# Rainbowboys/fm_spark

Measured on AMD Instinct MI355X. Metric: FM SGD train samples/sec at k=16, 1/8 GPUs; % of HBM roofline, higher is better.
Workload: dtype f32; 1 GPU; c3: synthetic hashed 100M features, 39 nnz/row, k=16, batch 256K; num_features=100000000, k=16, batch_rows_per_gpu=262144, global_batch=262144, launch=single

## Files before the change

### fm_spark_amd/csrc/fm_context.h

```cpp
#pragma once

#include <map>
#include <memory>
#include <utility>

#include "fm_internal.h"

namespace fmhip {

struct Pinned {
  void* p = nullptr;
  size_t bytes = 0;
  void ensure(size_t n) {
    if (n <= bytes && p) return;
    if (p) (void)hipHostFree(p);
    p = nullptr;
    FM_HIP_CHECK(hipHostMalloc(&p, n, hipHostMallocDefault));
    bytes = n;
  }
  void ensure_slack(size_t n) {
    if (n > bytes || !p) ensure(n + n / 8 + 4096);
  }
  ~Pinned() {
    if (p) (void)hipHostFree(p);
// ... 217 lines not shown
      }
      it->second.ms += ms;
      it->second.n += 1;
      free_events.push_back(pe.second.first);
      free_events.push_back(pe.second.second);
    }
    pending.clear();
  }

  void ensure_hist(int64_t need) {
    if (need <= hist_cap) return;
    int64_t c = std::max<int64_t>(4096, hist_cap);
    while (c < need) c *= 2;
    FM_HIP_CHECK(hipStreamSynchronize(stream));
    DevBuf nb;
    nb.ensure(sizeof(double) * 3 * c);
    FM_HIP_CHECK(hipMemset(nb.p, 0, sizeof(double) * 3 * c));
    if (hist_cap > 0)
      FM_HIP_CHECK(hipMemcpy(nb.p, loss_hist.p, sizeof(double) * 3 * hist_cap, hipMemcpyDeviceToDevice));
    loss_hist = std::move(nb);
    hist_cap = c;
  }

  ~fm_ctx() {
    group.reset();
    (void)hipSetDevice(cfg.device);
    if (stream) (void)hipStreamSynchronize(stream);
    if (copy_stream) (void)hipStreamSynchronize(copy_stream);
    for (auto& h : hslot) {
      if (h.copied) (void)hipEventDestroy(h.copied);
      if (h.consumed) (void)hipEventDestroy(h.consumed);
    }
    if (copy_stream) (void)hipStreamDestroy(copy_stream);
    for (auto& pe : pending) {
      (void)hipEventDestroy(pe.second.first);
      (void)hipEventDestroy(pe.second.second);
    }
    for (auto e : free_events) (void)hipEventDestroy(e);
    if (side) (void)hipStreamSynchronize(side);
    if (ev_fork) (void)hipEventDestroy(ev_fork);
    if (ev_join) (void)hipEventDestroy(ev_join);
    if (ev_upd_done) (void)hipEventDestroy(ev_upd_done);
    if (side_own) (void)hipStreamSynchronize(side_own);
    if (side_own) (void)hipStreamDestroy(side_own);
    rec.release();
    loss_hist.release();
    DevBuf* bufs[] = {&work.S, &work.yl, &work.loss_part, &work.part, &work.ucnt,
                      &work.sort.keys_a, &work.sort.keys_b, &work.sort.vals_a, &work.sort.vals_b,
                      &work.sort.counts, &work.sort.digit_tot, &side_sort.keys_a, &side_sort.keys_b,
                      &side_sort.vals_a, &side_sort.vals_b, &side_sort.counts, &side_sort.digit_tot,
                      &route_sort.keys_a, &route_sort.keys_b, &route_sort.vals_a, &route_sort.vals_b,
                      &route_sort.counts, &route_sort.digit_tot,
                      &sh_okey, &sh_mask, &sh_tcnt, &sh_tot, &sh_pay, &sh_skey, &sh_ent2, &repl_cnt,
                      &split_work.cnt, &split_work.off, &rank.sum_u, &rank.sum_c, &rank.cnt_u, &rank.cnt_c,
                      &rank.bias_u, &rank.bias_c, &rank.lkey, &rank.lidx, &rank.out_idx, &rank.out_score};
    for (auto* b : bufs) b->release();
    if (own_stream && stream) (void)hipStreamDestroy(stream);
  }
};


namespace fmhip {
void report_stale(hipError_t e);

template <class F>
int guarded(fm_ctx* ctx, F&& f) {
  if (!ctx) {
    set_error("null fm_ctx");
    return FM_ERR_ARG;
  }
  std::lock_guard<std::mutex> lk(ctx->mu);
  int prev_dev = -1;
  if (hipGetDevice(&prev_dev) != hipSuccess) prev_dev = -1;
  struct Restore {
    int d;
    ~Restore() {
      if (d >= 0) (void)hipSetDevice(d);
    }
  } restore{prev_dev};
  try {
    report_stale(hipGetLastError());
    FM_HIP_CHECK(hipSetDevice(ctx->cfg.device));
    return f();
  } catch (const Error& e) {
    set_error(e.msg);
    return e.code;
  } catch (const std::bad_alloc&) {
    set_error("host allocation failed");
    return FM_ERR_OOM;
  } catch (const std::exception& e) {
    set_error(e.what());
    return FM_ERR_HIP;
  } catch (...) {
    set_error("unknown error");
    return FM_ERR_HIP;
  }
}

template <class F>
int guarded_free(F&& f) {
  try {
    return f();
  } catch (const Error& e) {
    set_error(e.msg);
    return e.code;
  } catch (const std::bad_alloc&) {
    set_error("host allocation failed");
// ... 68 lines not shown
```

### fm_spark_amd/csrc/fm_forward.hip

```cpp
#include <atomic>

#include "fm_device.h"

namespace fmhip {

namespace {

constexpr int kFuseNS = 5;
constexpr int kPartialU = 4;
constexpr int kFwdTeam = 32, kFwdU = 2;
constexpr int kFwdUNarrow = 3;
constexpr int kFwdGrid = 8192;
constexpr int kFuseU = 5;

__device__ __forceinline__ void fill_row(const FwdOut& xo, int k, int g, int64_t e, float4& v, float& w) {
  const int c = 4 * g;
  v = make_float4(c + 0 < k ? gauss_draw(xo.fill_seed, e, c + 0, xo.fill_sd) : 0.f,
                  c + 1 < k ? gauss_draw(xo.fill_seed, e, c + 1, xo.fill_sd) : 0.f,
                  c + 2 < k ? gauss_draw(xo.fill_seed, e, c + 2, xo.fill_sd) : 0.f,
                  c + 3 < k ? gauss_draw(xo.fill_seed, e, c + 3, xo.fill_sd) : 0.f);
  w = gauss_draw(xo.fill_seed, e, -1, xo.fill_sd);
}

template <int GS, int RPP>
__device__ __forceinline__ void loss_grad_walk(const TableView& T, const uint32_t* __restrict__ col,
                                               const float* __restrict__ xs, int64_t e0, int64_t e1, int rs, int g,
                                               bool qok, double cumE, double yhat, double y, double a0, double a1,
                                               double a2, double a3, const FwdOut& xo) {
  const double d = yhat - y;
  const int k = T.k;
  for (int64_t e = e0 + rs; e < e1; e += RPP) {
    const uint32_t id = col[e];
    const double xd = (double)xs[e];
    const bool inr = id < (uint64_t)T.rows;
    const RowHdr h = inr ? *T.hdr(id) : RowHdr{0.f, -1, 0.0};
    float4 v = qok && inr ? reinterpret_cast<const float4*>(T.v(id))[g] : make_float4(0.f, 0.f, 0.f, 0.f);
    float w;
    current_row(h, v, w, cumE);
    if (xo.fill_sd > 0.0 && h.t < 0) fill_row(xo, k, g, e, v, w);
    if (g == 0) {
      if (h.t < 0) *xo.absent = 1;
      xo.pred[e] = yhat;
      xo.loss[e] = d * d;
      xo.dw[e] = xd;
    }
    double* out = xo.dv + e * k;
    const int c = 4 * g;
    if (c + 0 < k) out[c + 0] = a0 * xd - ((double)v.x * xd) * xd;
    if (c + 1 < k) out[c + 1] = a1 * xd - ((double)v.y * xd) * xd;
    if (c + 2 < k) out[c + 2] = a2 * xd - ((double)v.z * xd) * xd;
    if (c + 3 < k) out[c + 3] = a3 * xd - ((double)v.w * xd) * xd;
  }
}

struct SampleOut {
  float4 Sq;
  double rj, yh;
};
struct SingleGrad { double t, b, gw; };
__device__ __forceinline__ SingleGrad single_grad(const SampleOut& so, double xd) {
  return SingleGrad{xd * so.rj, (xd * xd) * so.rj, (xd - 1.0) * so.yh + so.rj};
}
__device__ __forceinline__ float4 single_quad(float4 v_raw, float acf, float4 Sq, const SingleGrad& sg,
                                              const StepParams& sp) {
  const double A[4] = {fma((double)Sq.x, sg.t, 0.0), fma((double)Sq.y, sg.t, 0.0), fma((double)Sq.z, sg.t, 0.0),
                       fma((double)Sq.w, sg.t, 0.0)};
  return upd_quad(v_raw, acf, A, sg.b, sp);
}

template <int GS, int TEAM, bool STASH>
struct SingletonStash {
  static_assert(!STASH || (GS <= 4 && TEAM >= 16), "the fused forward serves kp <= 16");
  static constexpr int RPP = TEAM / GS;
  static constexpr int TPB = kBlock / TEAM;
  static constexpr int NS = STASH ? kFuseNS : 1;
  static constexpr int MZ = STASH ? NS * RPP : 1;
  using LdsV = float4[STASH ? TPB : 1][MZ][STASH ? GS : 1];
  using LdsH = float4[STASH ? TPB : 1][MZ];
  using LdsId = uint32_t[STASH ? TPB : 1][MZ];
  static __device__ __forceinline__ LdsV& lds_v() { __shared__ LdsV a; return a; }
  static __device__ __forceinline__ LdsH& lds_h() { __shared__ LdsH a; return a; }
  static __device__ __forceinline__ LdsId& lds_id() { __shared__ LdsId a; return a; }
  const TableView& T;
  const int team, rs, g;
  const bool qok;
  const int span;
  int nst = 0;
  int pend = 0;

  __device__ __forceinline__ SingletonStash(const TableView& T_, int team_, int rs_, int g_, bool qok_)
      : T(T_), team(team_), rs(rs_), g(g_), qok(qok_), span(hdr_span(T_.kp)) {}

  __device__ __forceinline__ int neighbour_pend() const { return STASH && GS >= 2 ? __shfl_xor(pend, GS) : 0; }

  __device__ __forceinline__ void keep(const RowHdr& h, float4 v, float x, uint32_t id) {
    if (nst < NS) {
      const int i = rs + nst * RPP;
      lds_v()[team][i][g] = v;
      if (g == 0) {
        RowHdr hx = h;
        hx.t = __float_as_int(x);
        lds_h()[team][i] = *reinterpret_cast<const float4*>(&hx);
        lds_id()[team][i] = id;
      }
    }
    ++nst;
  }

  __device__ __forceinline__ void flush(int pp) {
    const int kp = T.kp;
    if constexpr (GS >= 2) {
      const bool even = (rs & 1) == 0;
      const int n = pend > pp ? pend : pp;
      for (int j = 0; j < n; ++j) {
#pragma unroll
        for (int pass = 0; pass < 2; ++pass) {
          const bool writer = even == (pass == 0);
          const int slot = (writer ? rs : rs ^ 1) + j * RPP;
          const bool live = j < (writer ? pend : pp);
          const uint32_t sid = live ? lds_id()[team][slot] : 0u;
          float* rec = T.v(sid);
          const float4 val = writer ? lds_v()[team][slot][g] : (g == 0 ? lds_h()[team][slot] : make_float4(0.f, 0.f, 0.f, 0.f));
          if (live && (writer ? qok : 4 * g < span)) st_row4(writer ? rec + 4 * g : rec + kp + 4 * g, val);
        }
      }
    } else {
      for (int j = 0; j < pend; ++j) {
        const int i = rs + j * RPP;
        float* rec = T.v(lds_id()[team][i]);
        if (qok) st_row4(rec + 4 * g, lds_v()[team][i][g]);
        for (int c = 4 * g; c < span; c += 4 * GS) st_row4(rec + kp + c, c == 0 ? lds_h()[team][i] : make_float4(0.f, 0.f, 0.f, 0.f));
      }
    }
    pend = 0;
  }

  __device__ __forceinline__ void update(const SampleOut& so, const StepParams& sp, const uint32_t* __restrict__ col,
                                         const float* __restrict__ xs, int64_t e0, int64_t e1) {
    const int zc = nst < NS ? nst : NS;
    for (int jj = 0; jj < zc; ++jj) {
      const int i = rs + jj * RPP;
      const float4 hq = lds_h()[team][i];
      const RowHdr h = *reinterpret_cast<const RowHdr*>(&hq);
      const double xd = (double)__int_as_float(h.t);
      const float acf = pending_l1(h, sp);
      const SingleGrad sg = single_grad(so, xd);
      if (qok) lds_v()[team][i][g] = single_quad(lds_v()[team][i][g], acf, so.Sq, sg, sp);
      if (g == 0) {
        const RowHdr o = next_hdr(upd_w_row(h, acf, 0.0 + sg.gw, sp), sp);
        lds_h()[team][i] = *reinterpret_cast<const float4*>(&o);
      }
    }
    pend = zc;
    const int kp = T.kp;
    int seen = 0;
    for (int64_t e = e0 + rs; nst > NS && e < e1; e += RPP) {
      const uint32_t id = col[e];
      const RowHdr h = *T.hdr(id);
      if (is_multi(h.t, sp.epoch)) continue;
      if (++seen <= NS) continue;
      const float4 vq = qok ? reinterpret_cast<const float4*>(T.v(id))[g] : make_float4(0.f, 0.f, 0.f, 0.f);
      const double xd = (double)xs[e];
      const float acf = pending_l1(h, sp);
      float* rec = T.v(id);
      const SingleGrad sg = single_grad(so, xd);
      if (qok) st_row4(rec + 4 * g, single_quad(vq, acf, so.Sq, sg, sp));
      for (int i = 4 * g; i < span; i += 4 * GS) {
        float4 hq = make_float4(0.f, 0.f, 0.f, 0.f);
        if (i == 0) {
          const RowHdr o = next_hdr(upd_w_row(h, acf, 0.0 + sg.gw, sp), sp);
          hq = *reinterpret_cast<const float4*>(&o);
        }
        st_row4(rec + kp + i, hq);
      }
    }
  }
};

template <int MODE, int GS>
constexpr int fwd_min_waves() { return MODE == kTrainFused && GS == 4 ? 4 : 1; }

template <int GS, int TEAM, int MODE, int U>
__global__ __launch_bounds__(kBlock) __attribute__((amdgpu_waves_per_eu(fwd_min_waves<MODE, GS>())))
void k_forward(TableView T, const int64_t* __restrict__ row_ptr, const uint32_t* __restrict__ col,
               const uint2* __restrict__ ent, const float* __restrict__ xs, const double* __restrict__ label, int64_t B,
               double w0, double cumE, float* __restrict__ S_out, float2* __restrict__ yl_out, int64_t sstr, int64_t ystr,
               double2* __restrict__ loss_part, FwdOut xo) {
  constexpr bool PARTIAL = MODE == kPartial || MODE == kPartial64;
  constexpr bool STASH = MODE == kTrainFused;
  constexpr bool SUMMARY = MODE == kSummary;
  using Stash = SingletonStash<GS, TEAM, STASH>;
  constexpr int RPP = TEAM / GS;
  constexpr int TPB = kBlock / TEAM;
  const int tid = threadIdx.x;
  const int tl = tid % TEAM;
  const int g = tl % GS;
  const int rs = tl / GS;
  const int kp = T.kp;
  const bool qok = g * 4 < kp;
  double loss_acc = 0.0, nloss = 0.0;

  __shared__ int64_t ch_base[PARTIAL ? kMaxChunkSources + 1 : 1], ch_start[PARTIAL ? kMaxChunkSources : 1];
  const bool chunked = PARTIAL && xo.ch_C > 1;
  int64_t Bl = B;
  if (chunked) {
    if (tid == 0) {
      int64_t acc = 0;
      for (int r = 0; r < xo.ch_R; ++r) {
        const int64_t p0 = xo.ch_off[r], P = xo.ch_off[r + 1] - p0;
        const int64_t lo = P * xo.ch_c / xo.ch_C, hi = P * (xo.ch_c + 1) / xo.ch_C;
        ch_start[r] = p0 + lo;
        ch_base[r] = acc;
        acc += hi - lo;
      }
      ch_base[xo.ch_R] = acc;
    }
    __syncthreads();
    Bl = ch_base[xo.ch_R];
  }

  Stash stash(T, tid / TEAM, rs, g, qok);

  for (int64_t sl = (int64_t)blockIdx.x * TPB + tid / TEAM; sl < Bl; sl += (int64_t)gridDim.x * TPB) {
    int64_t s = sl;
    if (chunked) {
      int r = 0;
      while (sl >= ch_base[r + 1]) ++r;
      s = ch_start[r] + (sl - ch_base[r]);
    }
    const int64_t e0 = row_ptr[s], e1 = row_ptr[s + 1];
    const double ys = MODE == kTrainFused ? label[s] : 0.0;
    double a0 = 0.0, a1 = 0.0, a2 = 0.0, a3 = 0.0, vv = 0.0, wx = 0.0;
    uint32_t npres = 0;
    const int pp_s = stash.neighbour_pend();
    if (STASH) {
      stash.nst = 0;
      if (e0 + rs >= e1) stash.flush(pp_s);
    }
    for (int64_t eb = e0 + rs; eb < e1; eb += U * RPP) {
      uint32_t id[U];
      float x[U];
      bool ok[U];
#pragma unroll
      for (int j = 0; j < U; ++j) {
        const int64_t e = eb + j * RPP;
        ok[j] = e < e1;
        if constexpr (MODE == kTrainFused) {
          id[j] = ok[j] ? col[e] : 0u;
          x[j] = ok[j] ? xs[e] : 0.f;
        } else {
          const int64_t ec = ok[j] ? e : e1 - 1;
          const uint32_t idl = col[ec];
          const float xl = PARTIAL ? __uint_as_float(ent[ec].y) : xs[ec];
          id[j] = ok[j] ? idl : 0u;
          if (MODE == kPredict || SUMMARY) ok[j] = ok[j] && id[j] < (uint64_t)T.rows;
          x[j] = ok[j] ? xl : 0.f;
        }
      }
      if (STASH && eb == e0 + rs) stash.flush(pp_s);
      RowHdr h[U];
      float4 v[U];
#pragma unroll
      for (int j = 0; j < U; ++j) {
        if (ok[j] && (MODE != kLossGrad || id[j] < (uint64_t)T.rows)) {
          h[j] = *T.hdr(id[j]);
          v[j] = qok ? reinterpret_cast<const float4*>(T.v(id[j]))[g] : make_float4(0.f, 0.f, 0.f, 0.f);
        } else {
          h[j] = RowHdr{0.f, -1, 0.0};
          v[j] = make_float4(0.f, 0.f, 0.f, 0.f);
        }
      }
#pragma unroll
      for (int j = 0; j < U; ++j) {
        if (STASH && ok[j] && !is_multi(h[j].t, xo.sp.epoch)) stash.keep(h[j], v[j], x[j], id[j]);
      }
#pragma unroll
      for (int j = 0; j < U; ++j) {
        float w;
        if ((MODE == kPredict || PARTIAL || SUMMARY) && g == 0 && h[j].t >= 0) ++npres;
        current_row(h[j], v[j], w, cumE);
        if (MODE == kLossGrad && xo.fill_sd > 0.0 && ok[j] && h[j].t < 0) fill_row(xo, T.k, g, eb + j * RPP, v[j], w);
        const double xd = x[j];
        a0 += (double)v[j].x * xd; a1 += (double)v[j].y * xd;
        a2 += (double)v[j].z * xd; a3 += (double)v[j].w * xd;
        const double v2 = (double)v[j].x * v[j].x + (double)v[j].y * v[j].y + (double)v[j].z * v[j].z +
                          (double)v[j].w * v[j].w;
        vv += v2 * xd * xd;
        if (g == 0) wx += (double)w * xd;
      }
    }
#pragma unroll
    for (int o = GS; o < TEAM; o <<= 1) {
      a0 += __shfl_xor(a0, o); a1 += __shfl_xor(a1, o);
      a2 += __shfl_xor(a2, o); a3 += __shfl_xor(a3, o);
    }
#pragma unroll
    for (int o = 1; o < TEAM; o <<= 1) {
      vv += __shfl_xor(vv, o);
      wx += __shfl_xor(wx, o);
      if (MODE == kPredict || PARTIAL || SUMMARY) npres += __shfl_xor(npres, o);
    }
    if (PARTIAL || SUMMARY) {
      if constexpr (MODE == kPartial64 || SUMMARY) {
        if (rs == 0 && qok) {
          double2* so = reinterpret_cast<double2*>(reinterpret_cast<double*>(S_out) + s * sstr + g * 4);
          so[0] = make_double2(a0, a1);
          so[1] = make_double2(a2, a3);
        }
        if (tl == 0) reinterpret_cast<double2*>(yl_out)[s * ystr] = make_double2(vv, wx);
      } else {
        if (rs == 0 && qok)
          *reinterpret_cast<float4*>(S_out + s * sstr + g * 4) = make_float4((float)a0, (float)a1, (float)a2, (float)a3);
        if (tl == 0) yl_out[s * ystr] = make_float2((float)vv, (float)wx);
      }
      if (tl == 0) {
        if (xo.pcount) xo.pcount[s] = npres;
      }
      continue;
    }
    double ss = qok ? a0 * a0 + a1 * a1 + a2 * a2 + a3 * a3 : 0.0;
#pragma unroll
    for (int o = 1; o < GS; o <<= 1) ss += __shfl_xor(ss, o);
    const double yhat = 0.5 * (ss - vv) + wx + w0;
    if (MODE == kPredict) {
      if (tl == 0) xo.pred[s] = npres == 0 ? w0 : fmin(fmax(yhat, xo.lo), xo.hi);
      continue;
    }
    if (MODE == kLossGrad) {
      loss_grad_walk<GS, RPP>(T, col, xs, e0, e1, rs, g, qok, cumE, yhat, label[s], a0, a1, a2, a3, xo);
      continue;
    }
    if (rs == 0 && qok)
      *reinterpret_cast<float4*>(S_out + s * sstr + g * 4) = make_float4((float)a0, (float)a1, (float)a2, (float)a3);
    if constexpr (STASH) {
      const float r32 = (float)(yhat - ys), yh32 = (float)yhat;
      const SampleOut so{make_float4((float)a0, (float)a1, (float)a2, (float)a3), (double)r32, (double)yh32};
      stash.update(so, xo.sp, col, xs, e0, e1);
    }
    if (tl == 0) {
      const double y = label[s];
      yl_out[s * ystr] = make_float2((float)(yhat - y), (float)yhat);
      if (e1 > e0) {
        const double d = yhat - y;
        loss_acc += d * d;
        nloss += 1.0;
      }
    }
  }
  if (STASH) stash.flush(stash.neighbour_pend());
  if constexpr (MODE == kTrain || MODE == kTrainFused) block_loss_partial(loss_acc, nloss, loss_part);
}

std::atomic<int64_t> g_grid_cap{0};
std::mutex g_log_mu;
std::vector<FwdLaunchRec> g_log;
int64_t g_logged = 0;

void log_launch(const FwdLaunchRec& r) {
  std::lock_guard<std::mutex> lk(g_log_mu);
  if ((int)g_log.size() < kFwdLogCap) g_log.push_back(r);
  ++g_logged;
}

template <int GS, int TEAM, int MODE, int U>
void launch_fwd_m(const TableView& T, const BatchDev& b, StepWork& w, const StepParams& p, hipStream_t st,
                  int64_t* nblk, float* partial_out, FwdOut xo) {
  constexpr bool PARTIAL = MODE == kPartial || MODE == kPartial64, TRAIN = MODE == kTrain || MODE == kTrainFused;
  constexpr int TPB = kBlock / TEAM;
  int64_t blocks = (b.n_rows + TPB - 1) / TPB;
  const int64_t cap = g_grid_cap.load(std::memory_order_relaxed);
  const int64_t grid = cap > 0 ? cap : kFwdGrid;
  if (blocks > grid) blocks = grid;
  if (blocks < 1) blocks = 1;
  *nblk = blocks;
  if (cap > 0) log_launch(FwdLaunchRec{MODE, GS, TEAM, U, PARTIAL ? xo.ch_c : 0, PARTIAL ? xo.ch_C : 1, blocks, b.n_rows});
  float* S_out = nullptr;
  float2* yl_out = nullptr;
  int64_t sstr = T.kp, ystr = 1;
  double2* loss_part = nullptr;
  if (PARTIAL) {
    S_out = partial_out;
    yl_out = MODE == kPartial64 ? reinterpret_cast<float2*>(reinterpret_cast<double*>(partial_out) + b.n_rows * T.kp)
                                : reinterpret_cast<float2*>(partial_out + b.n_rows * T.kp);
  }
  if (MODE == kSummary) {
    S_out = reinterpret_cast<float*>(xo.summary);
    yl_out = reinterpret_cast<float2*>(xo.summary + b.n_rows * T.kp);
  }
  if (TRAIN) {
    w.loss_part.ensure(sizeof(double2) * blocks);
    S_out = w.S.as<float>();
    yl_out = s_rec_yl(T.kp) ? reinterpret_cast<float2*>(w.S.as<float>() + T.kp) : w.yl.as<float2>();
    sstr = s_rec_floats(T.kp);
    ystr = s_rec_yl(T.kp) ? (int64_t)s_rec_floats(T.kp) / 2 : (int64_t)1;
    loss_part = w.loss_part.as<double2>();
    if (MODE == kTrainFused) xo.sp = p;
  }
  hipLaunchKernelGGL((k_forward<GS, TEAM, MODE, U>), dim3((unsigned)blocks), dim3(kBlock), 0, st, T,
                     b.row_ptr.as<int64_t>(), b.col.as<uint32_t>(), b.ent.as<uint2>(),
                     PARTIAL ? nullptr : b.xs.as<float>(), TRAIN || MODE == kLossGrad ? b.label.as<double>() : nullptr,
                     b.n_rows, p.w0, p.cumE, S_out, yl_out, sstr, ystr, loss_part, xo);
}
// ... 129 lines not shown
```

### fm_spark_amd/csrc/fm_internal.h

```cpp
#pragma once

#include <hip/hip_runtime.h>

#include <cstdint>
#include <mutex>
#include <string>
#include <vector>

#include "../../include/fm_hip.h"

namespace fmhip {

void set_error(const std::string& msg);

struct Error {
  int code;
  std::string msg;
};

#define FM_HIP_CHECK(expr)                                                            \
  do {                                                                                \
    hipError_t _e = (expr);                                                           \
    if (_e != hipSuccess)                                                             \
      throw ::fmhip::Error{_e == hipErrorOutOfMemory ? FM_ERR_OOM : FM_ERR_HIP,        \
// ... 132 lines not shown
  double m;
  int32_t epoch;
  double cumE;
  double cum_next;
  double w0;
};

enum FwdMode : int { kTrain = 0, kPartial = 1, kPredict = 2, kLossGrad = 3, kTrainFused = 4, kPartial64 = 5, kSummary = 6 };
struct FwdOut {
  int mode = kTrain;
  double lo = 0.0, hi = 0.0;
  double* pred = nullptr;
  double* loss = nullptr;
  double* dw = nullptr;
  double* dv = nullptr;
  int32_t* absent = nullptr;
  uint32_t* pcount = nullptr;
  double* summary = nullptr;
  const int64_t* ch_off = nullptr;
  int32_t ch_R = 0, ch_c = 0, ch_C = 1;
  double fill_sd = 0.0;
  uint64_t fill_seed = 0;
  StepParams sp{};
};
constexpr int kMaxChunkSources = 64;
void launch_forward(const TableView& T, const BatchDev& b, StepWork& w, const StepParams& p,
                    hipStream_t st, int64_t* n_fwd_blocks, float* partial_out = nullptr,
                    const FwdOut* pred = nullptr, bool partial_wide = false);
struct FwdLaunchRec {
  int32_t mode, gs, team, u;
  int32_t chunk, chunks;
  int64_t blocks, rows;
};
constexpr int kFwdLogCap = 256;
struct FwdConsts {
  int32_t grid, block, fuse_ns, fuse_u;
};
void set_forward_grid_cap(int64_t blocks);
void clear_forward_log();
int read_forward_log(FwdLaunchRec* out, int cap);
FwdConsts forward_consts();

struct SegSource {
  const float* S;
  int64_t s_stride;
  const float2* yl;
  int64_t yl_stride;
  const int64_t* n_dev = nullptr;
};
void launch_segment_update(const TableView& T, const BatchDev& b, StepWork& w, const StepParams& p,
                           const uint32_t* skeys, const uint2* sents, int64_t n_fwd_blocks,
                           double* stats_out, hipStream_t st, float* emit = nullptr, const int64_t* n_dev = nullptr);
struct SplitWork {
  DevBuf cnt, off;
};
void launch_split(const uint32_t* skeys, const uint2* sents, int64_t N, SplitWork& sw, uint32_t* mkeys, uint2* ments,
                  int64_t* n_out, hipStream_t st, const TableView& tag_T, int32_t epoch);
void launch_segment_update(const TableView& T, int64_t N, const SegSource& src, StepWork& w, const StepParams& p,
                           const uint32_t* skeys, const uint2* sents, int64_t n_loss_blocks, double* stats_out,
                           hipStream_t st, float* emit = nullptr);
constexpr int kReplApplyBlocks = 256 * 16;
constexpr int kLossPartBlocks = 256 * 8;
void launch_repl_apply(const TableView& T, const float* grad, const StepParams& p, uint32_t* blk_touched,
                       double* n_touched, hipStream_t st);

void launch_init_random(const TableView& T, const int32_t* ids, int64_t n, int64_t id_begin,
                        uint64_t seed, double sd, int32_t epoch, double cumE, hipStream_t st);
void launch_load_rows(const TableView& T, const int32_t* ids, int64_t n, const double* w,
                      const double* V, int32_t epoch, double cumE, hipStream_t st);
void launch_flush(const TableView& T, int32_t epoch, double cumE, hipStream_t st);
void launch_gather_rows(const TableView& T, const int32_t* ids, int64_t n, double cumE, double* w, double* V,
                        int8_t* present, hipStream_t st);
void launch_table_reset(const TableView& T, hipStream_t st);
void launch_predict(const TableView& T, const BatchDev& b, double cumE, double w0, double lo, double hi,
                    double* pred, hipStream_t st);
void launch_summary(const TableView& T, const BatchDev& b, double cumE, double* summary, uint32_t* present,
                    hipStream_t st);
void launch_init_entries(const TableView& T, const uint32_t* col, int64_t n, uint64_t seed, double sd,
                         int32_t epoch, double cumE, hipStream_t st);
void launch_loss_grad(const TableView& T, const BatchDev& b, double cumE, double w0, double* pred,
                      double* loss, double* dw, double* dv, int32_t* absent_flag, hipStream_t st,
                      double fill_sd = 0.0, uint64_t fill_seed = 0);
void launch_segment_sum(const uint32_t* skeys, const uint32_t* svals, int64_t n, const double* vecs,
                        int32_t k, uint32_t* run_index, int32_t* out_keys, double* out_sums,
                        int64_t* n_out_dev, hipStream_t st);
void launch_count_present(const TableView& T, int64_t* out, hipStream_t st);
struct CsrImage {
  int64_t* row_ptr;
  double* label;
  int32_t* xoff;
  uint32_t* col;
  float* x;
};
void launch_explode(const CsrImage& in, int64_t B, int64_t N, BatchDev& dst, hipStream_t st);
void launch_layout_splits(const CsrImage& src, const int64_t* order, const int64_t* row_ptr_in, const int64_t* split_rows,
                          int32_t n_splits, int64_t B, BatchDev& dst, int64_t* split_rp, hipStream_t st);

struct RankWork {
  DevBuf sum_u, sum_c;
  DevBuf cnt_u, cnt_c;
  DevBuf bias_u, bias_c;
  DevBuf lkey, lidx;
  DevBuf out_idx, out_score;
};
int rank_splits(int64_t C, int64_t U);
int64_t rank_ctx_tile(int splits, int n_top);
void launch_rank_bias(const double* summary, int64_t n, int kp, double* bias, hipStream_t st);
// ... 14 lines not shown
```

### fm_spark_amd/csrc/fm_update.hip

```cpp
#include <algorithm>
#include <cstdlib>

#include "fm_device.h"

namespace fmhip {

namespace {

constexpr int kWaveEnt = 256;
constexpr int kUpdD = 2;
constexpr int kUpdD4 = 1;
constexpr int kUpdD2 = 1;

struct SegArgs {
  TableView T;
  const uint32_t* skeys;
  const uint2* sents;
  int64_t N;
  const float* S;
  const float2* yl;
  int64_t s_stride;
  int64_t yl_stride;
  double* part;
  int64_t nranges;
// ... 502 lines not shown
       i += (int64_t)gridDim.x * kBlock / G) {
    const float* gr = grad + i * W;
    const float2 wt = *reinterpret_cast<const float2*>(gr + kp);
    if (wt.y == 0.f) continue;
    touched += g == 0 ? 1u : 0u;
    const RowHdr h = *T.hdr(i);
    const bool present = h.t >= 0;
    const double ac = present ? p.cumE - h.cum : 0.0;
    float4* rec = reinterpret_cast<float4*>(T.v(i));
    for (int q = g; q < nq; q += G) {
      float4 v = present ? rec[q] : make_float4(0.f, 0.f, 0.f, 0.f);
      if (ac > 0.0) v = shrink4(v, ac);
      const float4 d = reinterpret_cast<const float4*>(gr)[q];
      rec[q] = make_float4(upd_v(v.x, d.x, p), upd_v(v.y, d.y, p), upd_v(v.z, d.z, p), upd_v(v.w, d.w, p));
    }
    if (g == 0) {
      float w = present ? h.w : 0.f;
      if (ac > 0.0) w = shrink_f(w, ac);
      store_hdr(T, i, next_hdr(upd_w(w, (double)wt.x, p), p));
    }
  }
  __shared__ uint32_t wt[kBlock / 64];
#pragma unroll
  for (int o = 32; o > 0; o >>= 1) touched += __shfl_xor(touched, o);
  if ((threadIdx.x & 63) == 0) wt[threadIdx.x >> 6] = touched;
  __syncthreads();
  if (threadIdx.x == 0) {
    uint32_t t = 0;
    for (int w = 0; w < kBlock / 64; ++w) t += wt[w];
    blk_touched[blockIdx.x] = t;
  }
}

__global__ __launch_bounds__(kBlock) void k_sum_counts(const uint32_t* __restrict__ c, int64_t n, double* __restrict__ out) {
  __shared__ uint64_t ws[kBlock / 64];
  uint64_t t = 0;
  for (int64_t i = threadIdx.x; i < n; i += kBlock) t += c[i];
#pragma unroll
  for (int o = 32; o > 0; o >>= 1) t += __shfl_xor(t, o);
  if ((threadIdx.x & 63) == 0) ws[threadIdx.x >> 6] = t;
  __syncthreads();
  if (threadIdx.x == 0) {
    uint64_t a = 0;
    for (int w = 0; w < kBlock / 64; ++w) a += ws[w];
    *out = (double)a;
  }
}
}

constexpr int kSplitChunk = 1024;

constexpr int kSplitRows = kSplitChunk / 64;
constexpr uint32_t kSplitNone = 0xFFFFFFFFu;
struct SplitChunk {
  uint32_t key[kSplitRows];
  uint32_t multi = 0, first = 0;
};
__device__ __forceinline__ void split_chunk(const uint32_t* __restrict__ skeys, int64_t N, int64_t c, int lane,
                                            SplitChunk& sc) {
  const int64_t base = c * kSplitChunk;
#pragma unroll
  for (int r = 0; r < kSplitRows; ++r) {
    const int64_t p = base + r * 64 + lane;
    sc.key[r] = skeys[p < N ? p : N - 1];
  }
  const int64_t eb = lane == 0 ? (base > 0 ? base - 1 : 0) : (base + kSplitChunk < N ? base + kSplitChunk : N - 1);
  const uint32_t edge = skeys[eb];
  const uint32_t before = base > 0 ? __shfl(edge, 0) : kSplitNone;
  const uint32_t after = base + kSplitChunk < N ? __shfl(edge, 1) : kSplitNone;
#pragma unroll
  for (int r = 0; r < kSplitRows; ++r) {
    const int64_t p = base + r * 64 + lane;
    const uint32_t up = __shfl_up(sc.key[r], 1), dn = __shfl_down(sc.key[r], 1);
    const uint32_t pl = r > 0 ? __shfl(sc.key[r > 0 ? r - 1 : 0], 63) : before;
    const uint32_t nf = r + 1 < kSplitRows ? __shfl(sc.key[r + 1 < kSplitRows ? r + 1 : r], 0) : after;
    const uint32_t prev = lane == 0 ? pl : up;
    const uint32_t next = p + 1 >= N ? kSplitNone : (lane == 63 ? nf : dn);
    const bool valid = p < N;
    sc.multi |= (uint32_t)(valid && (prev == sc.key[r] || next == sc.key[r])) << r;
    sc.first |= (uint32_t)(valid && prev != sc.key[r]) << r;
  }
}

__global__ __launch_bounds__(kBlock) void k_split_count(const uint32_t* __restrict__ skeys, int64_t N,
                                                        uint2* __restrict__ cnt, int64_t nchunks, TableView T,
                                                        int32_t epoch) {
  const int lane = threadIdx.x & 63;
  const int64_t c = (int64_t)blockIdx.x * (kBlock / 64) + (threadIdx.x >> 6);
  if (c >= nchunks) return;
  SplitChunk sc;
  split_chunk(skeys, N, c, lane, sc);
  const uint32_t tag = sc.multi & sc.first;
  int32_t tv[kSplitRows];
#pragma unroll
  for (int r = 0; r < kSplitRows; ++r) tv[r] = T.hdr((tag >> r) & 1u ? sc.key[r] : 0u)->t;
#pragma unroll
  for (int r = 0; r < kSplitRows; ++r)
    if ((tag >> r) & 1u) T.hdr(sc.key[r])->t = multi_tag(epoch, tv[r] >= 0);
  uint32_t nm = 0, ns = 0;
  const int64_t base = c * kSplitChunk;
#pragma unroll
  for (int r = 0; r < kSplitRows; ++r) {
    const bool valid = base + r * 64 + lane < N;
    const bool m = (sc.multi >> r) & 1u;
    nm += (uint32_t)__popcll(__ballot(m));
    ns += (uint32_t)__popcll(__ballot(valid && !m));
  }
  if (lane == 0) cnt[c] = make_uint2(nm, ns);
}

constexpr int kSplitPer = 12;
constexpr int kSplitScanNT = 1024;
__global__ __launch_bounds__(kSplitScanNT) void k_split_scan(const uint2* __restrict__ cnt, int64_t nchunks,
                                                             int64_t* __restrict__ off, int64_t* __restrict__ n_out) {
  constexpr int NW = kSplitScanNT / 64;
  __shared__ int64_t wsum[NW], ssum[NW];
  const int lane = threadIdx.x & 63, wave = threadIdx.x >> 6;
  int64_t carry = 0, singles = 0;
  for (int64_t b = 0; b < nchunks; b += kSplitScanNT * kSplitPer) {
    const int64_t i0 = b + (int64_t)threadIdx.x * kSplitPer;
    uint2 v[kSplitPer];
#pragma unroll
    for (int j = 0; j < kSplitPer; ++j) v[j] = cnt[i0 + j < nchunks ? i0 + j : nchunks - 1];
#pragma unroll
    for (int j = 0; j < kSplitPer; ++j)
      if (i0 + j >= nchunks) v[j] = make_uint2(0u, 0u);
    int64_t t = 0, sg = 0;
#pragma unroll
    for (int j = 0; j < kSplitPer; ++j) {
      t += v[j].x;
      sg += v[j].y;
    }
    int64_t incl = t;
#pragma unroll
    for (int o = 1; o < 64; o <<= 1) {
      const int64_t u = __shfl_up(incl, o);
      if (lane >= o) incl += u;
    }
#pragma unroll
    for (int o = 32; o > 0; o >>= 1) sg += __shfl_xor(sg, o);
    if (lane == 63) wsum[wave] = incl;
    if (lane == 0) ssum[wave] = sg;
    __syncthreads();
    int64_t wpre = 0, tot = 0, stot = 0;
    for (int w = 0; w < NW; ++w) {
      wpre += w < wave ? wsum[w] : 0;
      tot += wsum[w];
      stot += ssum[w];
    }
    int64_t run = carry + wpre + incl - t;
#pragma unroll
    for (int j = 0; j < kSplitPer; ++j) {
      if (i0 + j < nchunks) off[i0 + j] = run;
      run += v[j].x;
    }
    carry += tot;
    singles += stot;
    __syncthreads();
  }
  if (threadIdx.x == 0) {
    n_out[0] = carry;
    n_out[1] = singles;
  }
}

__global__ __launch_bounds__(kBlock) void k_split_scatter(const uint32_t* __restrict__ skeys,
                                                          const uint2* __restrict__ sents, int64_t N,
                                                          const int64_t* __restrict__ off, int64_t nchunks,
                                                          uint32_t* __restrict__ mkeys, uint2* __restrict__ ments) {
  const int lane = threadIdx.x & 63;
  const int64_t c = (int64_t)blockIdx.x * (kBlock / 64) + (threadIdx.x >> 6);
  if (c >= nchunks) return;
  const uint64_t lt = lane == 0 ? 0ull : (~0ull >> (64 - lane));
  const int64_t base = c * kSplitChunk;
  uint2 en[kSplitRows];
#pragma unroll
  for (int r = 0; r < kSplitRows; ++r) {
    const int64_t p = base + r * 64 + lane;
    en[r] = sents[p < N ? p : N - 1];
  }
  int64_t o = off[c];
  SplitChunk sc;
  split_chunk(skeys, N, c, lane, sc);
#pragma unroll
  for (int r = 0; r < kSplitRows; ++r) {
    const bool m = (sc.multi >> r) & 1u;
    const uint64_t bm = __ballot(m);
    if (m) {
      const int64_t d = o + __popcll(bm & lt);
      mkeys[d] = sc.key[r];
      ments[d] = en[r];
    }
    o += __popcll(bm);
  }
}

void launch_split(const uint32_t* skeys, const uint2* sents, int64_t N, SplitWork& sw, uint32_t* mkeys, uint2* ments,
                  int64_t* n_out, hipStream_t st, const TableView& tag_T, int32_t epoch) {
  const int64_t nchunks = (N + kSplitChunk - 1) / kSplitChunk;
  sw.cnt.ensure_slack(sizeof(uint2) * (size_t)std::max<int64_t>(nchunks, 1));
  sw.off.ensure_slack(sizeof(int64_t) * (size_t)std::max<int64_t>(nchunks, 1));
  if (N <= 0) {
    FM_HIP_CHECK(hipMemsetAsync(n_out, 0, 2 * sizeof(int64_t), st));
    return;
  }
  const unsigned blocks = (unsigned)((nchunks + kBlock / 64 - 1) / (kBlock / 64));
  hipLaunchKernelGGL(k_split_count, dim3(blocks), dim3(kBlock), 0, st, skeys, N, sw.cnt.as<uint2>(), nchunks, tag_T,
                     epoch);
  hipLaunchKernelGGL(k_split_scan, dim3(1), dim3(kSplitScanNT), 0, st, sw.cnt.as<uint2>(), nchunks, sw.off.as<int64_t>(), n_out);
  hipLaunchKernelGGL(k_split_scatter, dim3(blocks), dim3(kBlock), 0, st, skeys, sents, N, sw.off.as<int64_t>(), nchunks,
                     mkeys, ments);
  FM_HIP_CHECK(hipGetLastError());
}
void launch_segment_update(const TableView& T, const BatchDev& b, StepWork& w, const StepParams& p,
                           const uint32_t* skeys, const uint2* sents, int64_t n_fwd_blocks,
                           double* stats_out, hipStream_t st, float* emit, const int64_t* n_dev) {
  SegSource src{w.S.as<float>(), s_rec_floats(T.kp),
                 s_rec_yl(T.kp) ? reinterpret_cast<const float2*>(w.S.as<float>() + T.kp) : w.yl.as<float2>(),
                 s_rec_yl(T.kp) ? s_rec_floats(T.kp) / 2 : 1};
  src.n_dev = n_dev;
  launch_segment_update(T, b.nnz, src, w, p, skeys, sents, n_fwd_blocks, stats_out, st, emit);
}

void launch_segment_update(const TableView& T, int64_t N, const SegSource& src, StepWork& w, const StepParams& p,
                           const uint32_t* skeys, const uint2* sents, int64_t n_fwd_blocks, double* stats_out,
                           hipStream_t st, float* emit) {
  const int64_t L = kWaveEnt;
  const int64_t nranges = (N + L - 1) / L;
  w.part.ensure(sizeof(double) * (size_t)(nranges > 0 ? nranges : 1) * 2 * (T.kp + 2));
  const int64_t per_block = (int64_t)kWaveEnt * (kBlock / 64);
  const int64_t ublocks = (N + per_block - 1) / per_block;
  w.ucnt.ensure(sizeof(uint32_t) * (size_t)(ublocks > 0 ? ublocks : 1));
  SegArgs a;
  a.T = T;
  a.skeys = skeys;
  a.sents = sents;
  a.N = N;
  a.S = src.S;
  a.yl = src.yl;
  a.s_stride = src.s_stride;
  a.yl_stride = src.yl_stride;
  a.part = w.part.as<double>();
  a.nranges = nranges;
  a.L = L;
  a.p = p;
  a.ucnt = w.ucnt.as<uint32_t>();
  a.emit = emit;
  a.n_dev = src.n_dev;
  if (ublocks > 0) {
    const dim3 grid((unsigned)ublocks), blk(kBlock);
    const int nq = T.kp / 4;
    if (nq <= 1) hipLaunchKernelGGL((k_segment_update<1, 1, kUpdD>), grid, blk, 0, st, a);
    else if (nq <= 2) hipLaunchKernelGGL((k_segment_update<2, 1, kUpdD2>), grid, blk, 0, st, a);
    else if (nq <= 4) hipLaunchKernelGGL((k_segment_update<4, 1, kUpdD4>), grid, blk, 0, st, a);
    else if (nq <= 8) hipLaunchKernelGGL((k_segment_update<8, 1, kUpdD>), grid, blk, 0, st, a);
    else if (nq <= 16) hipLaunchKernelGGL((k_segment_update<16, 1, kUpdD>), grid, blk, 0, st, a);
    else if (nq <= 32) hipLaunchKernelGGL((k_segment_update<16, 2, 2>), grid, blk, 0, st, a);
    else hipLaunchKernelGGL((k_segment_update<16, 4, 1>), grid, blk, 0, st, a);
    FM_HIP_CHECK(hipGetLastError());
  }
  int64_t cblocks = (nranges * 16 + kBlock - 1) / kBlock;
  if (cblocks < 1) cblocks = 1;
  hipLaunchKernelGGL(k_segment_combine, dim3((unsigned)cblocks), dim3(kBlock), 0, st, a,
                     w.loss_part.as<double2>(), n_fwd_blocks, ublocks, stats_out);
  FM_HIP_CHECK(hipGetLastError());
// ... 24 lines not shown
```

Before: 330.7 million samples/s.

## Replace single-block split scan with group atomics and compact singleton stash ranks

The split step drops its single-block scan kernel. Per-chunk counts are now atomically accumulated into per-group sums, and each scatter wave computes its own prefix from those group sums. A ping-pong pair of group buffers is used, and each scatter launch zeroes the buffer the next launch will use. The fused forward's singleton stash now compacts kept rows across the team using ballot ranks instead of per-lane slots, which removes the neighbour-pending shuffle and adds wave-level LDS syncs. The fused kernel also requests the min-waves occupancy attribute for GS=2. Risks are atomic contention and redundant prefix reads in the scatter, plus more ballots in the forward.

Result: no change. 333.4 million samples/s, median of 6 (+0.8%).

```diff
diff --git a/fm_spark_amd/csrc/fm_context.h b/fm_spark_amd/csrc/fm_context.h
--- a/fm_spark_amd/csrc/fm_context.h
+++ b/fm_spark_amd/csrc/fm_context.h
@@ -293,7 +293,7 @@
                       &route_sort.keys_a, &route_sort.keys_b, &route_sort.vals_a, &route_sort.vals_b,
                       &route_sort.counts, &route_sort.digit_tot,
                       &sh_okey, &sh_mask, &sh_tcnt, &sh_tot, &sh_pay, &sh_skey, &sh_ent2, &repl_cnt,
-                      &split_work.cnt, &split_work.off, &rank.sum_u, &rank.sum_c, &rank.cnt_u, &rank.cnt_c,
+                      &split_work.cnt, &split_work.gsum, &rank.sum_u, &rank.sum_c, &rank.cnt_u, &rank.cnt_c,
                       &rank.bias_u, &rank.bias_c, &rank.lkey, &rank.lidx, &rank.out_idx, &rank.out_score};
     for (auto* b : bufs) b->release();
     if (own_stream && stream) (void)hipStreamDestroy(stream);
diff --git a/fm_spark_amd/csrc/fm_forward.hip b/fm_spark_amd/csrc/fm_forward.hip
--- a/fm_spark_amd/csrc/fm_forward.hip
+++ b/fm_spark_amd/csrc/fm_forward.hip
@@ -1,4 +1,5 @@
 #include <atomic>
+#include <type_traits>
 
 #include "fm_device.h"
 
@@ -70,7 +71,7 @@
 
 template <int GS, int TEAM, bool STASH>
 struct SingletonStash {
-  static_assert(!STASH || (GS <= 4 && TEAM >= 16), "the fused forward serves kp <= 16");
+  static_assert(!STASH || (GS <= 4 && TEAM >= 16 && TEAM <= 64), "the fused forward serves kp <= 16");
   static constexpr int RPP = TEAM / GS;
   static constexpr int TPB = kBlock / TEAM;
   static constexpr int NS = STASH ? kFuseNS : 1;
@@ -81,6 +82,12 @@
   static __device__ __forceinline__ LdsV& lds_v() { __shared__ LdsV a; return a; }
   static __device__ __forceinline__ LdsH& lds_h() { __shared__ LdsH a; return a; }
   static __device__ __forceinline__ LdsId& lds_id() { __shared__ LdsId a; return a; }
+  using TeamMask = std::conditional_t<(TEAM > 32), uint64_t, uint32_t>;
+  static constexpr TeamMask group_lanes() {
+    TeamMask m = 0;
+    for (int i = 0; i < TEAM; i += GS) m |= (TeamMask)1 << i;
+    return m;
+  }
   const TableView& T;
   const int team, rs, g;
   const bool qok;
@@ -91,11 +98,17 @@
   __device__ __forceinline__ SingletonStash(const TableView& T_, int team_, int rs_, int g_, bool qok_)
       : T(T_), team(team_), rs(rs_), g(g_), qok(qok_), span(hdr_span(T_.kp)) {}
 
-  __device__ __forceinline__ int neighbour_pend() const { return STASH && GS >= 2 ? __shfl_xor(pend, GS) : 0; }
-
-  __device__ __forceinline__ void keep(const RowHdr& h, float4 v, float x, uint32_t id) {
-    if (nst < NS) {
-      const int i = rs + nst * RPP;
+  __device__ __forceinline__ void pass_ranks(bool single, int& below, int& all) const {
+    const TeamMask tb = (TeamMask)(__ballot(single) >> ((threadIdx.x & 63) & ~(TEAM - 1))) & group_lanes();
+    below = __popcll(tb & (((TeamMask)1 << (rs * GS)) - 1));
+    all = __popcll(tb);
+  }
+
+  __device__ __forceinline__ void keep(bool single, const RowHdr& h, float4 v, float x, uint32_t id) {
+    int below, all;
+    pass_ranks(single, below, all);
+    const int i = nst + below;
+    if (single && i < MZ) {
       lds_v()[team][i][g] = v;
       if (g == 0) {
         RowHdr hx = h;
@@ -104,20 +117,19 @@
         lds_id()[team][i] = id;
       }
     }
-    ++nst;
-  }
-
-  __device__ __forceinline__ void flush(int pp) {
+    nst += all;
+  }
+
+  __device__ __forceinline__ void flush() {
     const int kp = T.kp;
     if constexpr (GS >= 2) {
       const bool even = (rs & 1) == 0;
-      const int n = pend > pp ? pend : pp;
-      for (int j = 0; j < n; ++j) {
+      for (int j0 = 0; j0 < pend; j0 += RPP) {
 #pragma unroll
         for (int pass = 0; pass < 2; ++pass) {
           const bool writer = even == (pass == 0);
-          const int slot = (writer ? rs : rs ^ 1) + j * RPP;
-          const bool live = j < (writer ? pend : pp);
+          const int slot = j0 + (writer ? rs : rs ^ 1);
+          const bool live = slot < pend;
           const uint32_t sid = live ? lds_id()[team][slot] : 0u;
           float* rec = T.v(sid);
           const float4 val = writer ? lds_v()[team][slot][g] : (g == 0 ? lds_h()[team][slot] : make_float4(0.f, 0.f, 0.f, 0.f));
@@ -125,21 +137,21 @@
         }
       }
     } else {
-      for (int j = 0; j < pend; ++j) {
-        const int i = rs + j * RPP;
+      for (int i = rs; i < pend; i += RPP) {
         float* rec = T.v(lds_id()[team][i]);
         if (qok) st_row4(rec + 4 * g, lds_v()[team][i][g]);
         for (int c = 4 * g; c < span; c += 4 * GS) st_row4(rec + kp + c, c == 0 ? lds_h()[team][i] : make_float4(0.f, 0.f, 0.f, 0.f));
       }
     }
     pend = 0;
+    wave_lds_sync();
   }
 
   __device__ __forceinline__ void update(const SampleOut& so, const StepParams& sp, const uint32_t* __restrict__ col,
                                          const float* __restrict__ xs, int64_t e0, int64_t e1) {
-    const int zc = nst < NS ? nst : NS;
-    for (int jj = 0; jj < zc; ++jj) {
-      const int i = rs + jj * RPP;
+    const int zc = nst < MZ ? nst : MZ;
+    wave_lds_sync();
+    for (int i = rs; i < zc; i += RPP) {
       const float4 hq = lds_h()[team][i];
       const RowHdr h = *reinterpret_cast<const RowHdr*>(&hq);
       const double xd = (double)__int_as_float(h.t);
@@ -151,34 +163,43 @@
         lds_h()[team][i] = *reinterpret_cast<const float4*>(&o);
       }
     }
+    wave_lds_sync();
     pend = zc;
+    if (nst <= MZ) return;
     const int kp = T.kp;
     int seen = 0;
-    for (int64_t e = e0 + rs; nst > NS && e < e1; e += RPP) {
-      const uint32_t id = col[e];
+    for (int64_t eb = e0; eb < e1; eb += RPP) {
+      const int64_t e = eb + rs;
+      const bool ok = e < e1;
+      const uint32_t id = ok ? col[e] : 0u;
       const RowHdr h = *T.hdr(id);
-      if (is_multi(h.t, sp.epoch)) continue;
-      if (++seen <= NS) continue;
-      const float4 vq = qok ? reinterpret_cast<const float4*>(T.v(id))[g] : make_float4(0.f, 0.f, 0.f, 0.f);
-      const double xd = (double)xs[e];
-      const float acf = pending_l1(h, sp);
-      float* rec = T.v(id);
-      const SingleGrad sg = single_grad(so, xd);
-      if (qok) st_row4(rec + 4 * g, single_quad(vq, acf, so.Sq, sg, sp));
-      for (int i = 4 * g; i < span; i += 4 * GS) {
-        float4 hq = make_float4(0.f, 0.f, 0.f, 0.f);
-        if (i == 0) {
-          const RowHdr o = next_hdr(upd_w_row(h, acf, 0.0 + sg.gw, sp), sp);
-          hq = *reinterpret_cast<const float4*>(&o);
+      const bool single = ok && !is_multi(h.t, sp.epoch);
+      int below, all;
+      pass_ranks(single, below, all);
+      const bool over = single && seen + below >= MZ;
+      seen += all;
+      if (over) {
+        const float4 vq = qok ? reinterpret_cast<const float4*>(T.v(id))[g] : make_float4(0.f, 0.f, 0.f, 0.f);
+        const double xd = (double)xs[e];
+        const float acf = pending_l1(h, sp);
+        float* rec = T.v(id);
+        const SingleGrad sg = single_grad(so, xd);
+        if (qok) st_row4(rec + 4 * g, single_quad(vq, acf, so.Sq, sg, sp));
+        for (int i = 4 * g; i < span; i += 4 * GS) {
+          float4 hq = make_float4(0.f, 0.f, 0.f, 0.f);
+          if (i == 0) {
+            const RowHdr o = next_hdr(upd_w_row(h, acf, 0.0 + sg.gw, sp), sp);
+            hq = *reinterpret_cast<const float4*>(&o);
+          }
+          st_row4(rec + kp + i, hq);
         }
-        st_row4(rec + kp + i, hq);
       }
     }
   }
 };
 
 template <int MODE, int GS>
-constexpr int fwd_min_waves() { return MODE == kTrainFused && GS == 4 ? 4 : 1; }
+constexpr int fwd_min_waves() { return MODE == kTrainFused && (GS == 4 || GS == 2) ? 4 : 1; }
 
 template <int GS, int TEAM, int MODE, int U>
 __global__ __launch_bounds__(kBlock) __attribute__((amdgpu_waves_per_eu(fwd_min_waves<MODE, GS>())))
@@ -232,12 +253,11 @@
     const double ys = MODE == kTrainFused ? label[s] : 0.0;
     double a0 = 0.0, a1 = 0.0, a2 = 0.0, a3 = 0.0, vv = 0.0, wx = 0.0;
     uint32_t npres = 0;
-    const int pp_s = stash.neighbour_pend();
     if (STASH) {
       stash.nst = 0;
-      if (e0 + rs >= e1) stash.flush(pp_s);
-    }
-    for (int64_t eb = e0 + rs; eb < e1; eb += U * RPP) {
+      if (e0 >= e1) stash.flush();
+    }
+    for (int64_t eb = e0 + rs; (STASH ? eb - rs : eb) < e1; eb += U * RPP) {
       uint32_t id[U];
       float x[U];
       bool ok[U];
@@ -257,7 +277,11 @@
           x[j] = ok[j] ? xl : 0.f;
         }
       }
-      if (STASH && eb == e0 + rs) stash.flush(pp_s);
+      if (STASH && eb == e0 + rs) stash.flush();
+      if constexpr (STASH) {
+#pragma unroll
+        for (int j = 0; j < U; ++j) asm volatile("" ::"v"(id[j]));
+      }
       RowHdr h[U];
       float4 v[U];
 #pragma unroll
@@ -272,7 +296,7 @@
       }
 #pragma unroll
       for (int j = 0; j < U; ++j) {
-        if (STASH && ok[j] && !is_multi(h[j].t, xo.sp.epoch)) stash.keep(h[j], v[j], x[j], id[j]);
+        if constexpr (STASH) stash.keep(ok[j] && !is_multi(h[j].t, xo.sp.epoch), h[j], v[j], x[j], id[j]);
       }
 #pragma unroll
       for (int j = 0; j < U; ++j) {
@@ -347,7 +371,7 @@
       }
     }
   }
-  if (STASH) stash.flush(stash.neighbour_pend());
+  if (STASH) stash.flush();
   if constexpr (MODE == kTrain || MODE == kTrainFused) block_loss_partial(loss_acc, nloss, loss_part);
 }
 
diff --git a/fm_spark_amd/csrc/fm_internal.h b/fm_spark_amd/csrc/fm_internal.h
--- a/fm_spark_amd/csrc/fm_internal.h
+++ b/fm_spark_amd/csrc/fm_internal.h
@@ -208,7 +208,11 @@
                            const uint32_t* skeys, const uint2* sents, int64_t n_fwd_blocks,
                            double* stats_out, hipStream_t st, float* emit = nullptr, const int64_t* n_dev = nullptr);
 struct SplitWork {
-  DevBuf cnt, off;
+  DevBuf cnt;
+  DevBuf gsum;
+  int64_t gcap = 0;
+  int64_t used[2] = {0, 0};
+  int cur = 0;
 };
 void launch_split(const uint32_t* skeys, const uint2* sents, int64_t N, SplitWork& sw, uint32_t* mkeys, uint2* ments,
                   int64_t* n_out, hipStream_t st, const TableView& tag_T, int32_t epoch);
diff --git a/fm_spark_amd/csrc/fm_update.hip b/fm_spark_amd/csrc/fm_update.hip
--- a/fm_spark_amd/csrc/fm_update.hip
+++ b/fm_spark_amd/csrc/fm_update.hip
@@ -578,6 +578,11 @@
 
 constexpr int kSplitRows = kSplitChunk / 64;
 constexpr uint32_t kSplitNone = 0xFFFFFFFFu;
+constexpr int kSplitGroup = 64;
+constexpr int kSplitGroupPer = 4;
+__device__ __forceinline__ unsigned long long split_pack(uint32_t multi, uint32_t singles) {
+  return (unsigned long long)multi | ((unsigned long long)singles << 32);
+}
 struct SplitChunk {
   uint32_t key[kSplitRows];
   uint32_t multi = 0, first = 0;
@@ -609,8 +614,8 @@
 }
 
 __global__ __launch_bounds__(kBlock) void k_split_count(const uint32_t* __restrict__ skeys, int64_t N,
-                                                        uint2* __restrict__ cnt, int64_t nchunks, TableView T,
-                                                        int32_t epoch) {
+                                                        uint2* __restrict__ cnt, unsigned long long* __restrict__ gsum,
+                                                        int64_t nchunks, TableView T, int32_t epoch) {
   const int lane = threadIdx.x & 63;
   const int64_t c = (int64_t)blockIdx.x * (kBlock / 64) + (threadIdx.x >> 6);
   if (c >= nchunks) return;
@@ -632,71 +637,23 @@
     nm += (uint32_t)__popcll(__ballot(m));
     ns += (uint32_t)__popcll(__ballot(valid && !m));
   }
-  if (lane == 0) cnt[c] = make_uint2(nm, ns);
-}
-
-constexpr int kSplitPer = 12;
-constexpr int kSplitScanNT = 1024;
-__global__ __launch_bounds__(kSplitScanNT) void k_split_scan(const uint2* __restrict__ cnt, int64_t nchunks,
-                                                             int64_t* __restrict__ off, int64_t* __restrict__ n_out) {
-  constexpr int NW = kSplitScanNT / 64;
-  __shared__ int64_t wsum[NW], ssum[NW];
-  const int lane = threadIdx.x & 63, wave = threadIdx.x >> 6;
-  int64_t carry = 0, singles = 0;
-  for (int64_t b = 0; b < nchunks; b += kSplitScanNT * kSplitPer) {
-    const int64_t i0 = b + (int64_t)threadIdx.x * kSplitPer;
-    uint2 v[kSplitPer];
-#pragma unroll
-    for (int j = 0; j < kSplitPer; ++j) v[j] = cnt[i0 + j < nchunks ? i0 + j : nchunks - 1];
-#pragma unroll
-    for (int j = 0; j < kSplitPer; ++j)
-      if (i0 + j >= nchunks) v[j] = make_uint2(0u, 0u);
-    int64_t t = 0, sg = 0;
-#pragma unroll
-    for (int j = 0; j < kSplitPer; ++j) {
-      t += v[j].x;
-      sg += v[j].y;
-    }
-    int64_t incl = t;
-#pragma unroll
-    for (int o = 1; o < 64; o <<= 1) {
-      const int64_t u = __shfl_up(incl, o);
-      if (lane >= o) incl += u;
-    }
-#pragma unroll
-    for (int o = 32; o > 0; o >>= 1) sg += __shfl_xor(sg, o);
-    if (lane == 63) wsum[wave] = incl;
-    if (lane == 0) ssum[wave] = sg;
-    __syncthreads();
-    int64_t wpre = 0, tot = 0, stot = 0;
-    for (int w = 0; w < NW; ++w) {
-      wpre += w < wave ? wsum[w] : 0;
-      tot += wsum[w];
-      stot += ssum[w];
-    }
-    int64_t run = carry + wpre + incl - t;
-#pragma unroll
-    for (int j = 0; j < kSplitPer; ++j) {
-      if (i0 + j < nchunks) off[i0 + j] = run;
-      run += v[j].x;
-    }
-    carry += tot;
-    singles += stot;
-    __syncthreads();
-  }
-  if (threadIdx.x == 0) {
-    n_out[0] = carry;
-    n_out[1] = singles;
+  if (lane == 0) {
+    cnt[c] = make_uint2(nm, ns);
+    atomicAdd(gsum + c / kSplitGroup, split_pack(nm, ns));
   }
 }
 
 __global__ __launch_bounds__(kBlock) void k_split_scatter(const uint32_t* __restrict__ skeys,
                                                           const uint2* __restrict__ sents, int64_t N,
-                                                          const int64_t* __restrict__ off, int64_t nchunks,
-                                                          uint32_t* __restrict__ mkeys, uint2* __restrict__ ments) {
+                                                          const uint2* __restrict__ cnt,
+                                                          const unsigned long long* __restrict__ gsum,
+                                                          unsigned long long* __restrict__ znext, int64_t nz,
+                                                          int64_t nchunks, uint32_t* __restrict__ mkeys,
+                                                          uint2* __restrict__ ments, int64_t* __restrict__ n_out) {
   const int lane = threadIdx.x & 63;
   const int64_t c = (int64_t)blockIdx.x * (kBlock / 64) + (threadIdx.x >> 6);
   if (c >= nchunks) return;
+  for (int64_t i = c * 64 + lane; i < nz; i += nchunks * 64) znext[i] = 0ull;
   const uint64_t lt = lane == 0 ? 0ull : (~0ull >> (64 - lane));
   const int64_t base = c * kSplitChunk;
   uint2 en[kSplitRows];
@@ -705,9 +662,34 @@
     const int64_t p = base + r * 64 + lane;
     en[r] = sents[p < N ? p : N - 1];
   }
-  int64_t o = off[c];
+  const int64_t grp = c / kSplitGroup;
+  const int cl = (int)(c % kSplitGroup);
+  const bool last = c == nchunks - 1;
+  const uint2 below = cnt[grp * kSplitGroup + (lane <= cl ? lane : cl)];
+  int64_t pm = lane < cl ? below.x : 0u, ps = lane <= cl ? below.y : 0u;
+  for (int64_t g0 = 0; g0 < grp; g0 += 64 * kSplitGroupPer) {
+    unsigned long long gv[kSplitGroupPer];
+#pragma unroll
+    for (int j = 0; j < kSplitGroupPer; ++j) {
+      const int64_t gi = g0 + j * 64 + lane;
+      gv[j] = gsum[gi < grp ? gi : grp - 1];
+    }
+#pragma unroll
+    for (int j = 0; j < kSplitGroupPer; ++j)
+      if (g0 + j * 64 + lane < grp) {
+        pm += (int64_t)(gv[j] & 0xFFFFFFFFull);
+        ps += (int64_t)(gv[j] >> 32);
+      }
+  }
   SplitChunk sc;
   split_chunk(skeys, N, c, lane, sc);
+#pragma unroll
+  for (int o = 32; o > 0; o >>= 1) pm += __shfl_xor(pm, o);
+  if (last) {
+#pragma unroll
+    for (int o = 32; o > 0; o >>= 1) ps += __shfl_xor(ps, o);
+  }
+  int64_t o = pm;
 #pragma unroll
   for (int r = 0; r < kSplitRows; ++r) {
     const bool m = (sc.multi >> r) & 1u;
@@ -719,24 +701,42 @@
     }
     o += __popcll(bm);
   }
-}
+  if (last && lane == 0) {
+    n_out[0] = o;
+    n_out[1] = ps;
+  }
+}
+
+int64_t split_groups(int64_t nchunks) { return (nchunks + kSplitGroup - 1) / kSplitGroup; }
 
 void launch_split(const uint32_t* skeys, const uint2* sents, int64_t N, SplitWork& sw, uint32_t* mkeys, uint2* ments,
                   int64_t* n_out, hipStream_t st, const TableView& tag_T, int32_t epoch) {
   const int64_t nchunks = (N + kSplitChunk - 1) / kSplitChunk;
   sw.cnt.ensure_slack(sizeof(uint2) * (size_t)std::max<int64_t>(nchunks, 1));
-  sw.off.ensure_slack(sizeof(int64_t) * (size_t)std::max<int64_t>(nchunks, 1));
+  const int64_t ngroups = split_groups(std::max<int64_t>(nchunks, 1));
+  if (ngroups > sw.gcap || !sw.gsum.p) {
+    const int64_t cap = ngroups + ngroups / 8 + 512;
+    sw.gsum.ensure(sizeof(unsigned long long) * 2 * (size_t)cap);
+    FM_HIP_CHECK(hipMemsetAsync(sw.gsum.p, 0, sizeof(unsigned long long) * 2 * (size_t)cap, st));
+    sw.gcap = cap;
+    sw.used[0] = sw.used[1] = 0;
+    sw.cur = 0;
+  }
   if (N <= 0) {
     FM_HIP_CHECK(hipMemsetAsync(n_out, 0, 2 * sizeof(int64_t), st));
     return;
   }
+  unsigned long long* mine = sw.gsum.as<unsigned long long>() + (int64_t)sw.cur * sw.gcap;
+  unsigned long long* next = sw.gsum.as<unsigned long long>() + (int64_t)(sw.cur ^ 1) * sw.gcap;
   const unsigned blocks = (unsigned)((nchunks + kBlock / 64 - 1) / (kBlock / 64));
-  hipLaunchKernelGGL(k_split_count, dim3(blocks), dim3(kBlock), 0, st, skeys, N, sw.cnt.as<uint2>(), nchunks, tag_T,
-                     epoch);
-  hipLaunchKernelGGL(k_split_scan, dim3(1), dim3(kSplitScanNT), 0, st, sw.cnt.as<uint2>(), nchunks, sw.off.as<int64_t>(), n_out);
-  hipLaunchKernelGGL(k_split_scatter, dim3(blocks), dim3(kBlock), 0, st, skeys, sents, N, sw.off.as<int64_t>(), nchunks,
-                     mkeys, ments);
+  hipLaunchKernelGGL(k_split_count, dim3(blocks), dim3(kBlock), 0, st, skeys, N, sw.cnt.as<uint2>(), mine, nchunks,
+                     tag_T, epoch);
+  hipLaunchKernelGGL(k_split_scatter, dim3(blocks), dim3(kBlock), 0, st, skeys, sents, N, sw.cnt.as<uint2>(), mine, next,
+                     sw.used[sw.cur ^ 1], nchunks, mkeys, ments, n_out);
   FM_HIP_CHECK(hipGetLastError());
+  sw.used[sw.cur] = ngroups;
+  sw.used[sw.cur ^ 1] = 0;
+  sw.cur ^= 1;
 }
 void launch_segment_update(const TableView& T, const BatchDev& b, StepWork& w, const StepParams& p,
                            const uint32_t* skeys, const uint2* sents, int64_t n_fwd_blocks,
```
